# drprojects/superpoint_transformer

Measured on AMD Instinct MI355X. Metric: Mpoints/s SPT fwd+bwd on S3DIS-scale NAG, higher is better.
Workload: dtype f32 (the reference's shipped matmul class - configs/train.yaml:60-61 `float32_matmul_precision: high` = TF32 / bf16x3 next to `precision: 32` - as bf16x3: matrix products on the bf16 pipe with split operands, attention and the backward of the fused layers and of the attention blocks' Linears hi*hi +

## Files before the change

### superpoint_transformer_amd/csrc/fused_pool.hip

```cpp
#include <math.h>

#include <type_traits>

#include "common.hpp"

namespace spt {
namespace fpool {

typedef float f32x4 __attribute__((ext_vector_type(4)));
typedef __bf16 bf16x8 __attribute__((ext_vector_type(8)));
typedef __bf16 bf16x4 __attribute__((ext_vector_type(4)));
typedef short s16x4 __attribute__((ext_vector_type(4)));
#ifndef SPT_FPOOL_SKIP
#define SPT_FPOOL_SKIP 0
#endif
#ifndef SPT_FPOOL_WPAD
#define SPT_FPOOL_WPAD 16
#endif
constexpr int TR = 16;
constexpr int NWF = 8;
constexpr int ARG_NONE = 0x7fffffff;

__device__ __forceinline__ double xg_sum_d(double v) {
  v += __shfl_xor(v, 16, 64);
  v += __shfl_xor(v, 32, 64);
  return v;
}
__device__ __forceinline__ float xg_sum_f(float v) {
  v += __shfl_xor(v, 16, 64);
  v += __shfl_xor(v, 32, 64);
  return v;
}
__device__ __forceinline__ void wave_sync_lds() {
  __builtin_amdgcn_fence(__ATOMIC_RELEASE, "wavefront");
  __builtin_amdgcn_wave_barrier();
  __builtin_amdgcn_fence(__ATOMIC_ACQUIRE, "wavefront");
}
template <bool B16>
__device__ __forceinline__ float4 ld4(const float* __restrict__ base, int64_t elem) {
  if constexpr (B16) {
    const uint2 u = *reinterpret_cast<const uint2*>(reinterpret_cast<const uint16_t*>(base) + elem);
    return make_float4(__uint_as_float(u.x << 16), __uint_as_float(u.x & 0xffff0000u),
                       __uint_as_float(u.y << 16), __uint_as_float(u.y & 0xffff0000u));
  } else {
    return *reinterpret_cast<const float4*>(base + elem);
  }
}
template <int NV, typename V>
__device__ __forceinline__ void split2(const float (&x)[NV], V& hi, V& lo) {
#pragma unroll
  for (int i = 0; i < NV; ++i) {
    const __bf16 h = (__bf16)x[i];
    hi[i] = h;
    lo[i] = (__bf16)(x[i] - (float)h);
  }
}
template <int NV, typename V>
__device__ __forceinline__ void split3(const float (&x)[NV], V& h, V& m, V& l) {
#pragma unroll
  for (int i = 0; i < NV; ++i) {
    const __bf16 a = (__bf16)x[i];
    const float r1 = x[i] - (float)a;
    const __bf16 b = (__bf16)r1;
    const float r2 = r1 - (float)b;
    h[i] = a;
    m[i] = b;
    l[i] = (__bf16)r2;
  }
}
__device__ __forceinline__ f32x4 mfma16(const bf16x4& a, const bf16x4& b, f32x4 c) {
  return __builtin_amdgcn_mfma_f32_16x16x16bf16_1k(__builtin_bit_cast(s16x4, a),
                                                   __builtin_bit_cast(s16x4, b), c, 0, 0, 0);
}

template <bool X16>
struct RowChunk { typedef float4 type; };
template <>
struct RowChunk<true> { typedef uint2 type; };
template <bool X16>
__device__ __forceinline__ float4 widen(const typename RowChunk<X16>::type& u) {
  if constexpr (X16) {
    return make_float4(__uint_as_float(u.x << 16), __uint_as_float(u.x & 0xffff0000u),
                       __uint_as_float(u.y << 16), __uint_as_float(u.y & 0xffff0000u));
  } else {
    return u;
  }
}
template <int K, bool X16>
__device__ __forceinline__ void load_rows(const float* __restrict__ x, int rid_l,
                                          typename RowChunk<X16>::type (&v)[TR * (K / 4) / 64], int lane) {
  constexpr int CH = K / 4, NIT = TR * CH / 64;
  static_assert(TR * CH % 64 == 0, "whole waves of chunks");
#pragma unroll
  for (int j = 0; j < NIT; ++j) {
    const int q = lane + 64 * j, rr = q / CH, k = (q - rr * CH) << 2;
// ... 132 lines not shown
  };

  const int64_t nw = (int64_t)gridDim.x * NWF, w = (int64_t)blockIdx.x * NWF + wid;
  const int64_t per = (((r1 - r0 + nw - 1) / nw) + TR - 1) / TR * TR;
  const int64_t pa0 = cut_at(r0 + w * per, r0, r1, pos_seg, rowptr);
  const int64_t pb0 = (w == nw - 1) ? r1 : cut_at(r0 + (w + 1) * per, r0, r1, pos_seg, rowptr);
  const bool has_rows = pa0 < pb0;
  const int64_t plast = pb0 - 1;
  auto ids_of = [&](int64_t p, int& rid, int& sg) {
    int64_t q = p + (lane & (TR - 1));
    q = q < plast ? q : plast;
    rid = perm ? perm[q] : (int)q;
    sg = pos_seg[q];
  };
  if (has_rows) {
  int seg_a, seg_b, rid_c, seg_c;
  typename RowChunk<IN16>::type xv[TR * (K / 4) / 64];
  {
    int rid0, rid1;
    ids_of(pa0, rid0, seg_a);
    load_rows<K, IN16>(x, rid0, xv, lane);
    ids_of(pa0 + TR, rid1, seg_b);
    ids_of(pa0 + 2 * TR, rid_c, seg_c);
    wave_sync_lds();
    store_rows<K, LDA, true, IN16>(xv, (int)((pb0 - pa0) < TR ? (pb0 - pa0) : TR), tab, pslope, al, lane);
    load_rows<K, IN16>(x, rid1, xv, lane);
  }
  for (int64_t p = pa0; p < pb0; p += TR) {
    const int cnt = (int)((pb0 - p) < TR ? (pb0 - p) : TR);
    wave_sync_lds();
    f32x4 C[NBK];
#pragma unroll
    for (int nb = 0; nb < NBK; ++nb) C[nb] = (f32x4){0.f, 0.f, 0.f, 0.f};
    if constexpr (!(SPT_FPOOL_SKIP & 4)) {
      constexpr int NSTEP = KS * NBK;
      constexpr int LA = NPL == 3 ? 2 : (NPL == 2 ? 3 : 6);
      bf16x8 wf[LA + 1][NPL];
      auto ldw = [&](int step, bf16x8 (&w)[NPL]) {
        const int ks = step / NBK, nb = step - ks * NBK;
        const int wo = (16 * nb + c) * LDW + 32 * ks + 8 * g;
#pragma unroll
        for (int pl = 0; pl < NPL; ++pl) w[pl] = *reinterpret_cast<const bf16x8*>(&wpl[pl][wo]);
      };
#pragma unroll
      for (int i = 0; i < LA; ++i) ldw(i, wf[i]);
      bf16x8 x1, x2, x3;
#pragma unroll
      for (int step = 0; step < NSTEP; ++step) {
        const int ks = step / NBK, nb = step - ks * NBK;
        if (nb == 0) {
          const float4 a0 = *reinterpret_cast<const float4*>(al + c * LDA + 32 * ks + 8 * g);
          const float4 a1 = *reinterpret_cast<const float4*>(al + c * LDA + 32 * ks + 8 * g + 4);
          const float av[8] = {a0.x, a0.y, a0.z, a0.w, a1.x, a1.y, a1.z, a1.w};
          if constexpr (PREC == 3) {
            split3<8>(av, x1, x2, x3);
          } else if constexpr (PREC == 2) {
            split2<8>(av, x1, x2);
          } else {
#pragma unroll
            for (int i = 0; i < 8; ++i) x1[i] = (__bf16)av[i];
          }
        }
        if (step + LA < NSTEP) ldw(step + LA, wf[(step + LA) % (LA + 1)]);
        __builtin_amdgcn_sched_barrier(0);
        const bf16x8 (&w)[NPL] = wf[step % (LA + 1)];
        f32x4 acc = C[nb];
        if constexpr (PREC == 3) {
          acc = __builtin_amdgcn_mfma_f32_16x16x32_bf16(x3, w[0], acc, 0, 0, 0);
          acc = __builtin_amdgcn_mfma_f32_16x16x32_bf16(x1, w[NPL - 1], acc, 0, 0, 0);
          acc = __builtin_amdgcn_mfma_f32_16x16x32_bf16(x2, w[NPL > 1 ? 1 : 0], acc, 0, 0, 0);
          acc = __builtin_amdgcn_mfma_f32_16x16x32_bf16(x2, w[0], acc, 0, 0, 0);
          acc = __builtin_amdgcn_mfma_f32_16x16x32_bf16(x1, w[NPL > 1 ? 1 : 0], acc, 0, 0, 0);
        } else if constexpr (PREC == 2) {
          acc = __builtin_amdgcn_mfma_f32_16x16x32_bf16(x2, w[0], acc, 0, 0, 0);
          acc = __builtin_amdgcn_mfma_f32_16x16x32_bf16(x1, w[NPL - 1], acc, 0, 0, 0);
        }
        acc = __builtin_amdgcn_mfma_f32_16x16x32_bf16(x1, w[0], acc, 0, 0, 0);
        C[nb] = acc;
        __builtin_amdgcn_sched_barrier(0);
      }
    }
    if constexpr (!(SPT_FPOOL_SKIP & 1)) {
      bf16x4 Yh[KB], Yl[KB];
#pragma unroll
      for (int kb = 0; kb < KB; ++kb) {
        float yv[4];
#pragma unroll
        for (int r = 0; r < 4; ++r) yv[r] = al[(4 * g + r) * LDA + 16 * kb + c];
        if constexpr (PREC != 1) {
          const float sh = tab[3 * K + 16 * kb + c];
#pragma unroll
          for (int r = 0; r < 4; ++r) yv[r] = (4 * g + r < cnt) ? yv[r] - sh : 0.f;
        }
        if constexpr (PREC == 1) {
#pragma unroll
          for (int r = 0; r < 4; ++r) {
            Yh[kb][r] = (__bf16)yv[r];
            yv[r] = (float)Yh[kb][r];
          }
        } else {
          split2<4>(yv, Yh[kb], Yl[kb]);
        }
        sy[kb] += (yv[0] + yv[1]) + (yv[2] + yv[3]);
      }
      int gi = 0;
#pragma unroll
      for (int mi = 0; mi < KB; ++mi)
#pragma unroll
        for (int ni = mi; ni < KB; ++ni) {
          f32x4 acc = GA[gi];
          if constexpr (PREC != 1) {
            acc = mfma16(Yl[mi], Yl[ni], acc);
            acc = mfma16(Yl[mi], Yh[ni], acc);
            acc = mfma16(Yh[mi], Yl[ni], acc);
          }
          GA[gi] = mfma16(Yh[mi], Yh[ni], acc);
          ++gi;
        }
    }
    wave_sync_lds();
    {
      const int64_t left = pb0 - (p + TR);
      store_rows<K, LDA, true, IN16>(xv, (int)(left < 0 ? 0 : (left < TR ? left : TR)), tab, pslope, al, lane);
      asm volatile("" : "+v"(rid_c), "+v"(seg_c));
    }
    const int seg_cur = seg_a;
    if constexpr (!(SPT_FPOOL_SKIP & 2)) {
      const int pos0 = (int)p + 4 * g;
      int row = 0;
      while (row < cnt) {
        const int s = __builtin_amdgcn_readlane(seg_cur, row);
        const uint64_t diff = __ballot(lane < cnt && lane > row && seg_cur != s);
        const int e = diff ? (int)__builtin_ctzll(diff) : cnt;
        if (s != cur_seg) {
          if (cur_seg >= 0) flush(cur_seg);
          cur_seg = s;
        }
        if (row == 0 && e == TR) {
#pragma unroll
          for (int r = 0; r < 4; ++r)
#pragma unroll
            for (int nb = 0; nb < NBK; ++nb) {
              const float v = C[nb][r];
              const bool win = v > pm[nb];
              pm[nb] = win ? v : pm[nb];
              pp[nb] = win ? pos0 + r : pp[nb];
            }
        } else {
#pragma unroll
          for (int r = 0; r < 4; ++r) {
            const int rr = 4 * g + r;
            const bool in = rr >= row && rr < e;
#pragma unroll
            for (int nb = 0; nb < NBK; ++nb) {
              const float v = in ? C[nb][r] : -INFINITY;
              const bool win = v > pm[nb];
              pm[nb] = win ? v : pm[nb];
              pp[nb] = win ? pos0 + r : pp[nb];
            }
          }
        }
        row = e;
      }
    }
    load_rows<K, IN16>(x, rid_c, xv, lane);
    seg_a = seg_b;
    seg_b = seg_c;
    ids_of(p + 3 * TR, rid_c, seg_c);
  }
  }
  if (cur_seg >= 0) flush(cur_seg);

  for (int i = threadIdx.x; i < K * K + K; i += NWF * 64) gred[i] = 0.0;
  __syncthreads();
  for (int ww = 0; ww < NWF; ++ww) {
// ... 164 lines not shown
    const float* __restrict__ sc, const float* __restrict__ bs, float slope,
    const float* __restrict__ c1, float* __restrict__ gm) {
  const int64_t t4 = ((int64_t)blockIdx.x * blockDim.x + threadIdx.x) * 4;
  if (t4 >= num_seg * N) return;
  const int64_t s = t4 / N;
  const int c = (int)(t4 - s * N);
  const int64_t gph = seg_graph ? seg_graph[s] : 0;
  const float4 go = *reinterpret_cast<const float4*>(gout + t4);
  const float4 hv = *reinterpret_cast<const float4*>(raw + t4);
  const float4 a = *reinterpret_cast<const float4*>(am + gph * N + c);
  const float4 sv = *reinterpret_cast<const float4*>(sc + gph * N + c);
  const float4 b = *reinterpret_cast<const float4*>(bs + c);
  const float4 k1 = *reinterpret_cast<const float4*>(c1 + gph * N + c);
  const float gg[4] = {go.x, go.y, go.z, go.w}, hh[4] = {hv.x, hv.y, hv.z, hv.w};
  const float aa[4] = {a.x, a.y, a.z, a.w}, ss[4] = {sv.x, sv.y, sv.z, sv.w};
  const float bb[4] = {b.x, b.y, b.z, b.w}, q1[4] = {k1.x, k1.y, k1.z, k1.w};
  float o[4];
#pragma unroll
  for (int e = 0; e < 4; ++e) {
    float g_ = gg[e];
    if (slope != 1.f) {
      const float y = fmaf(hh[e] - aa[e], ss[e], bb[e]);
      g_ = (y > 0.f) ? g_ : g_ * slope;
    }
    o[e] = q1[e] * g_;
  }
  *reinterpret_cast<float4*>(gm + t4) = make_float4(o[0], o[1], o[2], o[3]);
}

template <int K>
__global__ __launch_bounds__(256) void pool_bwd_coef_kernel(
    const float* __restrict__ W, int N, const float* __restrict__ am, const float* __restrict__ c2,
    const float* __restrict__ c3, float* __restrict__ M, float* __restrict__ c0) {
  const int b = blockIdx.x;
  extern __shared__ float sm[];
  float* Bc = sm;
  float* Ac = sm + N;
  for (int i = threadIdx.x; i < N; i += blockDim.x) {
    const float k2 = c2[b * N + i];
    Bc[i] = -k2;
    Ac[i] = fmaf(k2, am[b * N + i], -c3[b * N + i]);
  }
  __syncthreads();
  for (int i = blockIdx.y * blockDim.x + threadIdx.x; i < K * K + K; i += gridDim.y * blockDim.x) {
    double acc = 0.0;
    if (i < K * K) {
      const int j = i / K, k = i - j * K;
      for (int c = 0; c < N; ++c)
        acc += (double)W[(size_t)c * K + j] * (double)Bc[c] * (double)W[(size_t)c * K + k];
      M[(size_t)b * K * K + i] = (float)acc;
    } else {
      const int k = i - K * K;
      for (int c = 0; c < N; ++c) acc += (double)Ac[c] * (double)W[(size_t)c * K + k];
      c0[(size_t)b * K + k] = (float)acc;
    }
  }
}

template <int K>
__global__ __launch_bounds__(256) void pool_bwd_gw_dense_kernel(
    const double* __restrict__ gram, int B, const float* __restrict__ W, int N, int bfw,
    const float* __restrict__ am, const float* __restrict__ c2, const float* __restrict__ c3,
    float* __restrict__ gW) {
  constexpr int GLEN = K * K + K + 1;
  const int t = blockIdx.x * blockDim.x + threadIdx.x;
  if (t >= N * K) return;
  const int c = t / K, k = t - c * K;
  double acc = 0.0;
  for (int b = 0; b < B; ++b) {
    const double* gr = gram + (size_t)b * GLEN;
    const double k2 = (double)c2[b * N + c];
    const double Ac = (double)fmaf(c2[b * N + c], am[b * N + c], -c3[b * N + c]);
    double t1 = 0.0;
    for (int j = 0; j < K; ++j) {
      float w = W[(size_t)c * K + j];
      if (bfw) w = (float)(__bf16)w;
      t1 += (double)w * gr[j * K + k];
    }
    acc += -k2 * t1 + Ac * gr[K * K + k];
  }
  gW[t] = (float)((double)gW[t] + acc);
}

template <int K, int N, bool LO, bool X16, int NW>
__global__ __launch_bounds__(NW * 64, NW / 4) void bwd_pool_kernel(
    const float* __restrict__ gm, const int32_t* __restrict__ argpos,
    const int32_t* __restrict__ perm, const int32_t* __restrict__ pos_seg,
    const float* __restrict__ xprev, const float* __restrict__ pam,
    const float* __restrict__ psc, const float* __restrict__ pbs, float pslope,
    const float* __restrict__ W, const float* __restrict__ Mg, const float* __restrict__ c0g,
    float* __restrict__ gx, float* __restrict__ gw_partial, double* __restrict__ pstat_partial,
    FmlpRuns rt) {
  constexpr int KB = K / 16, NBK = N / 16, NS = N / 32, KS = K / 32;
  constexpr int NBH = NBK / 2, KBH = KB / 2;
  constexpr int LDG = N + 4, LDX = K + 4;
  constexpr int LDT = N + SPT_FPOOL_WPAD, LDM = K + SPT_FPOOL_WPAD;
  static_assert((LDT % 32 == 16 && LDM % 32 == 16) || SPT_FPOOL_WPAD != 16, "conflict-free B fragments");
  constexpr int CPL = N / 64;
  static_assert(K % 32 == 0 && N % 64 == 0 && NW % 2 == 0, "shape");
  __shared__ __attribute__((aligned(16))) float g_lds[NW][TR * LDG];
  __shared__ __attribute__((aligned(16))) float x_lds[NW][TR * LDX];
  __shared__ __attribute__((aligned(16))) __bf16 wt_hi[K * LDT];
  __shared__ __attribute__((aligned(16))) __bf16 wt_lo[LO ? K * LDT : 8];
  __shared__ __attribute__((aligned(16))) __bf16 mt_hi[K * LDM];
  __shared__ __attribute__((aligned(16))) __bf16 mt_lo[LO ? K * LDM : 8];
  __shared__ __attribute__((aligned(16))) float pt[3 * K];
  __shared__ __attribute__((aligned(16))) float c0l[K];
  const int lane = threadIdx.x & 63;
  const int wid = __builtin_amdgcn_readfirstlane(threadIdx.x >> 6);
  const int hf = wid & 1;
  const int nb0 = hf * NBH, kb0 = hf * KBH;
  const int g = lane >> 4, c = lane & 15;
  const int run = blockIdx.y, gph = rt.g[run];
  const int64_t r0 = rt.r0[run], r1 = rt.r1[run];
  pam += (size_t)gph * K;
  psc += (size_t)gph * K;
  Mg += (size_t)gph * K * K;
  c0g += (size_t)gph * K;
  constexpr int SCR = 4 * (K / 32) * 64;
  float* gw_scratch = gw_partial + (size_t)gridDim.y * gridDim.x * N * K +
                      (size_t)run * gridDim.x * (NW / 2) * 2 * SCR;
  gw_partial += (size_t)run * gridDim.x * N * K;
  pstat_partial += (size_t)run * gridDim.x * (NW / 2) * (2 * K + 1);
  float* gl = g_lds[wid];
  float* xl = x_lds[wid];
  for (int i = threadIdx.x; i < K * N; i += NW * 64) {
    const int k = i / N, n = i - k * N;
    const float w = W[(size_t)n * K + k];
    const __bf16 hh = (__bf16)w;
    wt_hi[k * LDT + n] = hh;
    if constexpr (LO) wt_lo[k * LDT + n] = (__bf16)(w - (float)hh);
  }
  for (int i = threadIdx.x; i < K * K; i += NW * 64) {
    const int k = i / K, j = i - k * K;
    const float m = Mg[(size_t)j * K + k];
    const __bf16 hh = (__bf16)m;
    mt_hi[k * LDM + j] = hh;
    if constexpr (LO) mt_lo[k * LDM + j] = (__bf16)(m - (float)hh);
  }
  for (int i = threadIdx.x; i < K; i += NW * 64) {
    pt[i] = pam[i];
    pt[K + i] = psc[i];
    pt[2 * K + i] = pbs[i];
    c0l[i] = c0g[i];
  }
  __syncthreads();

  f32x4 C3[NBH][KB];
#pragma unroll
  for (int nb = 0; nb < NBH; ++nb)
#pragma unroll
    for (int kb = 0; kb < KB; ++kb) C3[nb][kb] = (f32x4){0.f, 0.f, 0.f, 0.f};
  double p1[KBH], p2[KBH];
#pragma unroll
  for (int kb = 0; kb < KBH; ++kb) p1[kb] = p2[kb] = 0.0;

  const int64_t ntiles = (r1 - r0 + TR - 1) / TR;
  const int64_t pair = (int64_t)blockIdx.x * (NW / 2) + (wid >> 1);
  const int64_t npairs = (int64_t)gridDim.x * (NW / 2);
  auto cnt_of = [&](int64_t t) {
    const int64_t row0 = r0 + t * TR;
    return (t < ntiles) ? (int)((r1 - row0) < TR ? (r1 - row0) : TR) : 0;
  };
  auto load_ids = [&](int64_t t, int& rid, int& sg) {
    const int64_t tt = t < ntiles ? t : ntiles - 1;
    int64_t q = r0 + tt * TR + (lane & (TR - 1));
    q = q < r1 - 1 ? q : r1 - 1;
    rid = perm ? perm[q] : (int)q;
    sg = pos_seg[q];
  };
  auto load_seg = [&](int sgm, int (&ap)[CPL], float (&gv)[CPL]) {
    const size_t o = (size_t)sgm * N + CPL * lane;
    if constexpr (CPL == 2) {
      const int2 a2 = *reinterpret_cast<const int2*>(argpos + o);
      const float2 g2 = *reinterpret_cast<const float2*>(gm + o);
      ap[0] = a2.x; ap[1] = a2.y;
      gv[0] = g2.x; gv[1] = g2.y;
    } else {
      ap[0] = argpos[o];
      gv[0] = gm[o];
    }
  };
  auto scatter = [&](const int (&ap)[CPL], const float (&gv)[CPL], int row0i, int lo, int hi) {
#pragma unroll
    for (int q = 0; q < CPL; ++q) {
      const int rr = ap[q] - row0i;
      const bool ok = rr >= lo && rr < hi;
      gl[ok ? rr * LDG + CPL * lane + q : N + q] = gv[q];
    }
  };
  if (ntiles > 0) {
  int rid_l, seg_l, rid_n, seg_n;
  load_ids(pair, rid_l, seg_l);
  typename RowChunk<X16>::type xv[TR * (K / 4) / 64];
  load_rows<K, X16>(xprev, rid_l, xv, lane);
  int apA[CPL], apB[CPL];
  float gvA[CPL], gvB[CPL];
  {
    const int c0 = cnt_of(pair < ntiles ? pair : ntiles - 1);
    load_seg(__builtin_amdgcn_readlane(seg_l, 0), apA, gvA);
    load_seg(__builtin_amdgcn_readlane(seg_l, c0 - 1), apB, gvB);
  }
  load_ids(pair + npairs, rid_n, seg_n);
  {
    float* scratch = gw_scratch + ((size_t)pair * 2 + hf) * SCR;
#pragma unroll
    for (int i = 0; i < 4 * KBH; ++i) scratch[lane + 64 * i] = 0.f;
  }
  auto tile = [&](auto full_c, int64_t t) {
    constexpr bool FULL = decltype(full_c)::value;
    const int64_t row0 = r0 + t * TR;
    const int cnt = FULL ? TR : cnt_of(t);
    wave_sync_lds();
    store_rows<K, LDX, false, X16>(xv, cnt, nullptr, 1.f, xl, lane);
    {
      constexpr int NZ = TR * (N / 4) / 64;
#pragma unroll
      for (int j = 0; j < NZ; ++j) {
        const int q = lane + 64 * j, rr = q / (N / 4), n = (q - rr * (N / 4)) << 2;
        *reinterpret_cast<float4*>(gl + rr * LDG + n) = make_float4(0.f, 0.f, 0.f, 0.f);
      }
      const int sA = __builtin_amdgcn_readlane(seg_l, 0);
      const int sB = __builtin_amdgcn_readlane(seg_l, cnt - 1);
      const uint64_t notA = __ballot(lane < cnt && seg_l != sA);
      const int eA = notA ? (int)__builtin_ctzll(notA) : cnt;
      const uint64_t isB = __ballot(lane < cnt && seg_l == sB);
      const int bB = (int)__builtin_ctzll(isB);
      scatter(apA, gvA, (int)row0, 0, eA);
      if (sB != sA) scatter(apB, gvB, (int)row0, bB, cnt);
      int row = eA;
      while (row < bB) {
        const int sgm = __builtin_amdgcn_readlane(seg_l, row);
        const uint64_t diff = __ballot(lane < cnt && lane > row && seg_l != sgm);
        const int e = diff ? (int)__builtin_ctzll(diff) : cnt;
        int ap[CPL];
        float gv[CPL];
        load_seg(sgm, ap, gv);
        scatter(ap, gv, (int)row0, row, e);
        row = e;
      }
    }
    const int rid_cur = rid_l;
    load_rows<K, X16>(xprev, rid_n, xv, lane);
    {
      const int64_t tn = t + npairs < ntiles ? t + npairs : ntiles - 1;
      load_seg(__builtin_amdgcn_readlane(seg_n, 0), apA, gvA);
      load_seg(__builtin_amdgcn_readlane(seg_n, cnt_of(tn) - 1), apB, gvB);
    }
    rid_l = rid_n;
    seg_l = seg_n;
    load_ids(t + 2 * npairs, rid_n, seg_n);
    wave_sync_lds();
    auto ynorm = [&](float v, int k, bool ok) {
      v = fmaf(v - pt[k], pt[K + k], pt[2 * K + k]);
      v = (v > 0.f) ? v : v * pslope;
      return ok ? v : 0.f;
    };
    if constexpr (!(SPT_FPOOL_SKIP & 8)) {
      bf16x4 Xh[KB], Xl[KB];
#pragma unroll
      for (int kb = 0; kb < KB; ++kb) {
        const int k = 16 * kb + c;
        float xr4[4];
#pragma unroll
        for (int r = 0; r < 4; ++r) xr4[r] = ynorm(xl[(4 * g + r) * LDX + k], k, 4 * g + r < cnt);
        if constexpr (LO) {
          split2<4>(xr4, Xh[kb], Xl[kb]);
        } else {
#pragma unroll
          for (int r = 0; r < 4; ++r) Xh[kb][r] = (__bf16)xr4[r];
        }
      }
#pragma unroll
      for (int nb = 0; nb < NBH; ++nb) {
        float sv[4];
#pragma unroll
        for (int r = 0; r < 4; ++r) sv[r] = gl[(4 * g + r) * LDG + 16 * (nb0 + nb) + c];
        bf16x4 sh, sl;
        if constexpr (LO) {
          split2<4>(sv, sh, sl);
        } else {
#pragma unroll
          for (int r = 0; r < 4; ++r) sh[r] = (__bf16)sv[r];
        }
#pragma unroll
        for (int kb = 0; kb < KB; ++kb) {
          f32x4 acc = C3[nb][kb];
          if constexpr (LO) {
            acc = mfma16(sl, Xh[kb], acc);
            acc = mfma16(sh, Xl[kb], acc);
          }
          C3[nb][kb] = mfma16(sh, Xh[kb], acc);
        }
      }
    }
    {
      f32x4 CX[KBH];
#pragma unroll
      for (int kb = 0; kb < KBH; ++kb) {
        const float z = c0l[16 * (kb0 + kb) + c];
        CX[kb] = (f32x4){z, z, z, z};
      }
      constexpr int NPLB = LO ? 2 : 1, LAB = 2;
      constexpr int NST1 = NS * KBH, NST = NST1 + KS * KBH;
      bf16x8 bf[LAB + 1][NPLB];
      auto ldb = [&](int step, bf16x8 (&b)[NPLB]) {
        if (step < NST1) {
          const int sg = step / KBH, kb = step - sg * KBH;
          const int wo = (16 * (kb0 + kb) + c) * LDT + 32 * sg + 8 * g;
          b[0] = *reinterpret_cast<const bf16x8*>(wt_hi + wo);
          if constexpr (LO) b[NPLB - 1] = *reinterpret_cast<const bf16x8*>(wt_lo + wo);
        } else {
          const int st = step - NST1, ks = st / KBH, kb = st - ks * KBH;
          const int mo = (16 * (kb0 + kb) + c) * LDM + 32 * ks + 8 * g;
          b[0] = *reinterpret_cast<const bf16x8*>(mt_hi + mo);
          if constexpr (LO) b[NPLB - 1] = *reinterpret_cast<const bf16x8*>(mt_lo + mo);
        }
      };
#pragma unroll
      for (int i = 0; i < LAB; ++i) ldb(i, bf[i]);
      bf16x8 ah, alo;
#pragma unroll
      for (int step = 0; step < ((SPT_FPOOL_SKIP & 16) ? 0 : NST); ++step) {
        const bool first = step < NST1;
        const int sub = first ? step : step - NST1;
        const int blk = sub / KBH, kb = sub - blk * KBH;
        if (kb == 0) {
          float av[8];
          if (first) {
            const float4 a0 = *reinterpret_cast<const float4*>(gl + c * LDG + 32 * blk + 8 * g);
            const float4 a1 = *reinterpret_cast<const float4*>(gl + c * LDG + 32 * blk + 8 * g + 4);
            av[0] = a0.x; av[1] = a0.y; av[2] = a0.z; av[3] = a0.w;
            av[4] = a1.x; av[5] = a1.y; av[6] = a1.z; av[7] = a1.w;
          } else {
            const float4 a0 = *reinterpret_cast<const float4*>(xl + c * LDX + 32 * blk + 8 * g);
            const float4 a1 = *reinterpret_cast<const float4*>(xl + c * LDX + 32 * blk + 8 * g + 4);
            const float rv[8] = {a0.x, a0.y, a0.z, a0.w, a1.x, a1.y, a1.z, a1.w};
#pragma unroll
            for (int i = 0; i < 8; ++i) av[i] = ynorm(rv[i], 32 * blk + 8 * g + i, c < cnt);
          }
          if constexpr (LO) {
            split2<8>(av, ah, alo);
          } else {
#pragma unroll
            for (int i = 0; i < 8; ++i) ah[i] = (__bf16)av[i];
          }
        }
        if (step + LAB < NST) ldb(step + LAB, bf[(step + LAB) % (LAB + 1)]);
        __builtin_amdgcn_sched_barrier(0);
        const bf16x8 (&b)[NPLB] = bf[step % (LAB + 1)];
        f32x4 acc = CX[kb];
        if constexpr (LO) {
          acc = __builtin_amdgcn_mfma_f32_16x16x32_bf16(alo, b[0], acc, 0, 0, 0);
          acc = __builtin_amdgcn_mfma_f32_16x16x32_bf16(ah, b[NPLB - 1], acc, 0, 0, 0);
        }
        CX[kb] = __builtin_amdgcn_mfma_f32_16x16x32_bf16(ah, b[0], acc, 0, 0, 0);
        __builtin_amdgcn_sched_barrier(0);
      }
#pragma unroll
      for (int r = 0; r < 4; ++r) {
        const int rr = 4 * g + r;
        const int64_t orow = (int64_t)__shfl(rid_cur, rr, 64);
        if (FULL || rr < cnt) {
#pragma unroll
          for (int kb = 0; kb < KBH; ++kb) {
            const int k = 16 * (kb0 + kb) + c;
            const float v = CX[kb][r];
            gx[orow * K + k] = v;
            const float o = xl[rr * LDX + k] - pt[k];
            float gg = v;
            if (pslope != 1.f) {
              const float y = fmaf(o, pt[K + k], pt[2 * K + k]);
              gg = (y > 0.f) ? gg : gg * pslope;
            }
            if constexpr (!(SPT_FPOOL_SKIP & 32)) {
              p1[kb] += (double)gg;
              p2[kb] += (double)gg * (double)o;
            }
          }
        }
      }
    }
  };
  const int64_t nfull = (r1 - r0) / TR;
  int64_t t = pair;
  for (; t < nfull; t += npairs) tile(std::true_type{}, t);
  if (t < ntiles) tile(std::false_type{}, t);
  }
  double* pp = pstat_partial + (size_t)pair * (2 * K + 1);
#pragma unroll
  for (int kb = 0; kb < KBH; ++kb) {
    const double a = xg_sum_d(p1[kb]), b = xg_sum_d(p2[kb]);
    const int k = 16 * (kb0 + kb) + c;
    if (g == 0) {
      pp[k] = a;
      pp[K + k] = b;
    }
  }
  if (lane == 0 && hf == 0) pp[2 * K] = (pair == 0) ? (double)(r1 - r0) : 0.0;
  {
    constexpr int LDR = K + 4;
    static_assert(N * LDR <= NW * TR * LDG, "the table fits the S-tile buffers");
    const int pr = wid >> 1;
    __syncthreads();
    float* red = &g_lds[0][0];
#pragma unroll 1
    for (int p = 1; p < NW / 2; ++p) {
      if (pr == p) {
#pragma unroll
        for (int nb = 0; nb < NBH; ++nb)
#pragma unroll
          for (int kb = 0; kb < KB; ++kb)
#pragma unroll
            for (int r = 0; r < 4; ++r)
              red[(16 * (nb0 + nb) + 4 * g + r) * LDR + 16 * kb + c] = C3[nb][kb][r];
      }
      __syncthreads();
      if (pr == 0) {
#pragma unroll
        for (int nb = 0; nb < NBH; ++nb)
#pragma unroll
          for (int kb = 0; kb < KB; ++kb)
#pragma unroll
            for (int r = 0; r < 4; ++r)
              C3[nb][kb][r] += red[(16 * (nb0 + nb) + 4 * g + r) * LDR + 16 * kb + c];
      }
      __syncthreads();
    }
    if (pr == 0) {
      float* gwp = gw_partial + (size_t)blockIdx.x * N * K;
#pragma unroll
      for (int nb = 0; nb < NBH; ++nb)
#pragma unroll
        for (int kb = 0; kb < KB; ++kb)
#pragma unroll
          for (int r = 0; r < 4; ++r)
            gwp[(size_t)(16 * (nb0 + nb) + 4 * g + r) * K + 16 * kb + c] = C3[nb][kb][r];
    }
  }
}

}

#define SPT_FPOOL_SHAPES(X) X(64, 128) X(64, 64) X(32, 64)

bool fpool_supported(int K, int N) {
#define X(k, n) if (K == k && N == n) return true;
  SPT_FPOOL_SHAPES(X)
#undef X
  return false;
}
int fpool_gram_len(int K) { return K * K + K + 1; }

int fpool_fwd_blocks(int64_t max_rows, int nruns) {
  int64_t blocks = (max_rows + fpool::TR * fpool::NWF * 4 - 1) / (fpool::TR * fpool::NWF * 4);
  int64_t cap = 256 / nruns;
  if (cap < 1) cap = 1;
  if (blocks > cap) blocks = cap;
  return (int)(blocks < 1 ? 1 : blocks);
}

int fpool_fwd_launch(int prec, bool in16, const float* x, const int32_t* perm, const int32_t* pos_seg,
                     const int32_t* rowptr, const FmlpRuns& rt, int64_t max_rows, int K, int N,
                     const float* W, const float* gnw, const float* pam, const float* psc,
                     const float* pbs, float pslope, float* raw, int32_t* argpos, double* partial,
                     hipStream_t stream) {
  const int gx_ = fpool_fwd_blocks(max_rows, rt.n);
  const dim3 grid((unsigned)gx_, (unsigned)rt.n);
#define X(k, n)                                                                                   \
  if (K == k && N == n) {                                                                         \
    if (prec == 3 && !in16)                                                                       \
      fpool::fwd_pool_kernel<k, n, 3, false><<<grid, fpool::NWF * 64, 0, stream>>>(               \
          x, perm, pos_seg, rowptr, W, gnw, pam, psc, pbs, pslope, raw, argpos, partial, rt);        \
    else if (prec == 2 && !in16)                                                                  \
      fpool::fwd_pool_kernel<k, n, 2, false><<<grid, fpool::NWF * 64, 0, stream>>>(               \
          x, perm, pos_seg, rowptr, W, gnw, pam, psc, pbs, pslope, raw, argpos, partial, rt);        \
    else if (prec == 1 && !in16)                                                                  \
      fpool::fwd_pool_kernel<k, n, 1, false><<<grid, fpool::NWF * 64, 0, stream>>>(               \
          x, perm, pos_seg, rowptr, W, gnw, pam, psc, pbs, pslope, raw, argpos, partial, rt);        \
    else if (prec == 1 && in16)                                                                   \
      fpool::fwd_pool_kernel<k, n, 1, true><<<grid, fpool::NWF * 64, 0, stream>>>(                \
          x, perm, pos_seg, rowptr, W, gnw, pam, psc, pbs, pslope, raw, argpos, partial, rt);        \
    else                                                                                          \
      return -1;                                                                                  \
  }
  SPT_FPOOL_SHAPES(X)
#undef X
  return gx_;
// ... 91 lines not shown
```

Baseline: 349.6.

## Store scattered pool gradient tile as split bf16 in LDS and read with transpose loads

The backward pool kernel used to scatter gradients into an fp32 LDS tile and re-split them into bf16 hi/lo on every read. It now splits once at scatter time into adjacent hi/lo bf16 halves of each row and reads fragments with ds_read_tr16_b64 transpose loads. In the C3 accumulation, the two correction MFMAs become one K=32 MFMA over concatenated lo/hi operands. A small forward tweak also replaces a row-masking select with an FMA against a row-valid factor. These cut LDS bytes, conversion ALU work and MFMA count, at the cost of a new LDS layout and reliance on the transpose-load intrinsic.

```diff
diff --git a/superpoint_transformer_amd/csrc/fused_pool.hip b/superpoint_transformer_amd/csrc/fused_pool.hip
--- a/superpoint_transformer_amd/csrc/fused_pool.hip
+++ b/superpoint_transformer_amd/csrc/fused_pool.hip
@@ -11,6 +11,7 @@
 typedef __bf16 bf16x8 __attribute__((ext_vector_type(8)));
 typedef __bf16 bf16x4 __attribute__((ext_vector_type(4)));
 typedef short s16x4 __attribute__((ext_vector_type(4)));
+typedef __attribute__((address_space(3))) s16x4 lds_s16x4;
 #ifndef SPT_FPOOL_SKIP
 #define SPT_FPOOL_SKIP 0
 #endif
@@ -309,6 +310,9 @@
     }
     if constexpr (!(SPT_FPOOL_SKIP & 1)) {
       bf16x4 Yh[KB], Yl[KB];
+      float rowin[4];
+#pragma unroll
+      for (int r = 0; r < 4; ++r) rowin[r] = (4 * g + r < cnt) ? 1.f : 0.f;
 #pragma unroll
       for (int kb = 0; kb < KB; ++kb) {
         float yv[4];
@@ -317,7 +321,7 @@
         if constexpr (PREC != 1) {
           const float sh = tab[3 * K + 16 * kb + c];
 #pragma unroll
-          for (int r = 0; r < 4; ++r) yv[r] = (4 * g + r < cnt) ? yv[r] - sh : 0.f;
+          for (int r = 0; r < 4; ++r) yv[r] = fmaf(-sh, rowin[r], yv[r]);
         }
         if constexpr (PREC == 1) {
 #pragma unroll
@@ -659,12 +663,14 @@
     FmlpRuns rt) {
   constexpr int KB = K / 16, NBK = N / 16, NS = N / 32, KS = K / 32;
   constexpr int NBH = NBK / 2, KBH = KB / 2;
-  constexpr int LDG = N + 4, LDX = K + 4;
+  constexpr int LDX = K + 4;
   constexpr int LDT = N + SPT_FPOOL_WPAD, LDM = K + SPT_FPOOL_WPAD;
   static_assert((LDT % 32 == 16 && LDM % 32 == 16) || SPT_FPOOL_WPAD != 16, "conflict-free B fragments");
+  constexpr int NPS = LO ? 2 : 1, LDS_ = NPS * N + 16;
+  static_assert(LDS_ % 32 == 16, "conflict-free S reads");
   constexpr int CPL = N / 64;
   static_assert(K % 32 == 0 && N % 64 == 0 && NW % 2 == 0, "shape");
-  __shared__ __attribute__((aligned(16))) float g_lds[NW][TR * LDG];
+  __shared__ __attribute__((aligned(16))) __bf16 s_lds[NW][TR * LDS_];
   __shared__ __attribute__((aligned(16))) float x_lds[NW][TR * LDX];
   __shared__ __attribute__((aligned(16))) __bf16 wt_hi[K * LDT];
   __shared__ __attribute__((aligned(16))) __bf16 wt_lo[LO ? K * LDT : 8];
@@ -688,7 +694,7 @@
                       (size_t)run * gridDim.x * (NW / 2) * 2 * SCR;
   gw_partial += (size_t)run * gridDim.x * N * K;
   pstat_partial += (size_t)run * gridDim.x * (NW / 2) * (2 * K + 1);
-  float* gl = g_lds[wid];
+  __bf16* sl_ = s_lds[wid];
   float* xl = x_lds[wid];
   for (int i = threadIdx.x; i < K * N; i += NW * 64) {
     const int k = i / N, n = i - k * N;
@@ -752,7 +758,10 @@
     for (int q = 0; q < CPL; ++q) {
       const int rr = ap[q] - row0i;
       const bool ok = rr >= lo && rr < hi;
-      gl[ok ? rr * LDG + CPL * lane + q : N + q] = gv[q];
+      const int o = ok ? rr * LDS_ + CPL * lane + q : NPS * N + 2 * q;
+      const __bf16 h = (__bf16)gv[q];
+      sl_[o] = h;
+      if constexpr (LO) sl_[o + (ok ? N : 1)] = (__bf16)(gv[q] - (float)h);
     }
   };
   if (ntiles > 0) {
@@ -780,11 +789,11 @@
     wave_sync_lds();
     store_rows<K, LDX, false, X16>(xv, cnt, nullptr, 1.f, xl, lane);
     {
-      constexpr int NZ = TR * (N / 4) / 64;
+      constexpr int CHR = NPS * N / 8, NZ = TR * CHR / 64;
 #pragma unroll
       for (int j = 0; j < NZ; ++j) {
-        const int q = lane + 64 * j, rr = q / (N / 4), n = (q - rr * (N / 4)) << 2;
-        *reinterpret_cast<float4*>(gl + rr * LDG + n) = make_float4(0.f, 0.f, 0.f, 0.f);
+        const int q = lane + 64 * j, rr = q / CHR, n = (q - rr * CHR) << 3;
+        *reinterpret_cast<uint4*>(sl_ + rr * LDS_ + n) = make_uint4(0u, 0u, 0u, 0u);
       }
       const int sA = __builtin_amdgcn_readlane(seg_l, 0);
       const int sB = __builtin_amdgcn_readlane(seg_l, cnt - 1);
@@ -837,26 +846,31 @@
           for (int r = 0; r < 4; ++r) Xh[kb][r] = (__bf16)xr4[r];
         }
       }
+      bf16x8 XX[LO ? KB : 1];
+      if constexpr (LO) {
+#pragma unroll
+        for (int kb = 0; kb < KB; ++kb)
+          XX[kb] = __builtin_shufflevector(Xh[kb], Xl[kb], 0, 1, 2, 3, 4, 5, 6, 7);
+      }
+      const __bf16* str = sl_ + (4 * g + (c >> 2)) * LDS_ + 4 * (c & 3);
+      auto tr_read = [&](int off) {
+        return __builtin_bit_cast(bf16x4, __builtin_amdgcn_ds_read_tr16_b64_v4i16(
+            (lds_s16x4*)(__attribute__((address_space(3))) void*)(str + off)));
+      };
 #pragma unroll
       for (int nb = 0; nb < NBH; ++nb) {
-        float sv[4];
-#pragma unroll
-        for (int r = 0; r < 4; ++r) sv[r] = gl[(4 * g + r) * LDG + 16 * (nb0 + nb) + c];
-        bf16x4 sh, sl;
+        const bf16x4 sh = tr_read(16 * (nb0 + nb));
         if constexpr (LO) {
-          split2<4>(sv, sh, sl);
+          const bf16x4 slo = tr_read(N + 16 * (nb0 + nb));
+          const bf16x8 SS = __builtin_shufflevector(slo, sh, 0, 1, 2, 3, 4, 5, 6, 7);
+#pragma unroll
+          for (int kb = 0; kb < KB; ++kb) {
+            const f32x4 acc = __builtin_amdgcn_mfma_f32_16x16x32_bf16(SS, XX[kb], C3[nb][kb], 0, 0, 0);
+            C3[nb][kb] = mfma16(sh, Xh[kb], acc);
+          }
         } else {
 #pragma unroll
-          for (int r = 0; r < 4; ++r) sh[r] = (__bf16)sv[r];
-        }
-#pragma unroll
-        for (int kb = 0; kb < KB; ++kb) {
-          f32x4 acc = C3[nb][kb];
-          if constexpr (LO) {
-            acc = mfma16(sl, Xh[kb], acc);
-            acc = mfma16(sh, Xl[kb], acc);
-          }
-          C3[nb][kb] = mfma16(sh, Xh[kb], acc);
+          for (int kb = 0; kb < KB; ++kb) C3[nb][kb] = mfma16(sh, Xh[kb], C3[nb][kb]);
         }
       }
     }
@@ -892,24 +906,23 @@
         const int sub = first ? step : step - NST1;
         const int blk = sub / KBH, kb = sub - blk * KBH;
         if (kb == 0) {
-          float av[8];
           if (first) {
-            const float4 a0 = *reinterpret_cast<const float4*>(gl + c * LDG + 32 * blk + 8 * g);
-            const float4 a1 = *reinterpret_cast<const float4*>(gl + c * LDG + 32 * blk + 8 * g + 4);
-            av[0] = a0.x; av[1] = a0.y; av[2] = a0.z; av[3] = a0.w;
-            av[4] = a1.x; av[5] = a1.y; av[6] = a1.z; av[7] = a1.w;
+            const __bf16* sr = sl_ + c * LDS_ + 32 * blk + 8 * g;
+            ah = *reinterpret_cast<const bf16x8*>(sr);
+            if constexpr (LO) alo = *reinterpret_cast<const bf16x8*>(sr + N);
           } else {
             const float4 a0 = *reinterpret_cast<const float4*>(xl + c * LDX + 32 * blk + 8 * g);
             const float4 a1 = *reinterpret_cast<const float4*>(xl + c * LDX + 32 * blk + 8 * g + 4);
             const float rv[8] = {a0.x, a0.y, a0.z, a0.w, a1.x, a1.y, a1.z, a1.w};
+            float av[8];
 #pragma unroll
             for (int i = 0; i < 8; ++i) av[i] = ynorm(rv[i], 32 * blk + 8 * g + i, c < cnt);
-          }
-          if constexpr (LO) {
-            split2<8>(av, ah, alo);
-          } else {
-#pragma unroll
-            for (int i = 0; i < 8; ++i) ah[i] = (__bf16)av[i];
+            if constexpr (LO) {
+              split2<8>(av, ah, alo);
+            } else {
+#pragma unroll
+              for (int i = 0; i < 8; ++i) ah[i] = (__bf16)av[i];
+            }
           }
         }
         if (step + LAB < NST) ldb(step + LAB, bf[(step + LAB) % (LAB + 1)]);
@@ -966,10 +979,10 @@
   if (lane == 0 && hf == 0) pp[2 * K] = (pair == 0) ? (double)(r1 - r0) : 0.0;
   {
     constexpr int LDR = K + 4;
-    static_assert(N * LDR <= NW * TR * LDG, "the table fits the S-tile buffers");
+    static_assert(2 * N * LDR <= NW * TR * LDS_, "the table fits the S-tile buffers");
     const int pr = wid >> 1;
     __syncthreads();
-    float* red = &g_lds[0][0];
+    float* red = reinterpret_cast<float*>(&s_lds[0][0]);
 #pragma unroll 1
     for (int p = 1; p < NW / 2; ++p) {
       if (pr == p) {
```

Measured after the change: 353.6, median of 6. 1.2% higher.

## Share pre-split bf16 tile planes between wave pairs via LDS flags in pool backward

Applied to the files above, without the earlier changes.

The backward pool kernel now has the two waves of a pair split the staging of each tile: each wave loads half the rows and half the channels, normalizes and splits them into swizzled bf16 hi/lo planes in a shared per-pair LDS record, and the pair synchronizes through LDS flag spin-waits. The MFMA operands are then read with ds_read_tr16 transpose loads, and hi/lo pairs are packed into a single 16x16x32 MFMA plus a 16x16x16 one, replacing three separate 16x16x16 MFMAs. The aim is to cut the redundant per-wave fp32 staging, the repeated ynorm and split work, and the LDS footprint. In exchange it adds inter-wave spin synchronization, with a trap if a wait times out, and it rounds S to bf16 before the MFMAs.

```diff
diff --git a/superpoint_transformer_amd/csrc/fused_pool.hip b/superpoint_transformer_amd/csrc/fused_pool.hip
--- a/superpoint_transformer_amd/csrc/fused_pool.hip
+++ b/superpoint_transformer_amd/csrc/fused_pool.hip
@@ -648,6 +648,36 @@
   gW[t] = (float)((double)gW[t] + acc);
 }
 
+typedef __attribute__((address_space(3))) s16x4 lds_s16x4;
+typedef __attribute__((address_space(3))) volatile int lds_flag_t;
+__device__ __forceinline__ void flag_set(lds_flag_t* f, int v) {
+  asm volatile("s_waitcnt lgkmcnt(0)" ::: "memory");
+  *f = v;
+}
+__device__ __forceinline__ bool flag_wait(lds_flag_t* f, int v) {
+  int spins = 0;
+  bool ok = true;
+#pragma clang loop unroll(disable)
+  while (__builtin_amdgcn_readfirstlane(*f) < v) {
+    __builtin_amdgcn_s_sleep(1);
+    if (++spins > (1 << 22)) {
+      ok = false;
+      break;
+    }
+  }
+  asm volatile("" ::: "memory");
+  return ok;
+}
+template <int C>
+__device__ __forceinline__ int pl_off(int row, int col) {
+  constexpr int RPL = 128 / C;
+  static_assert(C == 32 || C == 64 || C == 128, "plane row of 64, 128 or 256 bytes");
+  const int swz = ((row / RPL) & (8 / RPL - 1)) << 1;
+  return row * C + ((((col >> 3) ^ swz) << 3) | (col & 7));
+}
+__device__ __forceinline__ s16x4 tr_read(const __bf16* p) {
+  return __builtin_amdgcn_ds_read_tr16_b64_v4i16((lds_s16x4*)(__attribute__((address_space(3))) void*)p);
+}
 template <int K, int N, bool LO, bool X16, int NW>
 __global__ __launch_bounds__(NW * 64, NW / 4) void bwd_pool_kernel(
     const float* __restrict__ gm, const int32_t* __restrict__ argpos,
@@ -659,13 +689,27 @@
     FmlpRuns rt) {
   constexpr int KB = K / 16, NBK = N / 16, NS = N / 32, KS = K / 32;
   constexpr int NBH = NBK / 2, KBH = KB / 2;
-  constexpr int LDG = N + 4, LDX = K + 4;
+  constexpr int LDX = K + 4;
   constexpr int LDT = N + SPT_FPOOL_WPAD, LDM = K + SPT_FPOOL_WPAD;
   static_assert((LDT % 32 == 16 && LDM % 32 == 16) || SPT_FPOOL_WPAD != 16, "conflict-free B fragments");
-  constexpr int CPL = N / 64;
   static_assert(K % 32 == 0 && N % 64 == 0 && NW % 2 == 0, "shape");
-  __shared__ __attribute__((aligned(16))) float g_lds[NW][TR * LDG];
-  __shared__ __attribute__((aligned(16))) float x_lds[NW][TR * LDX];
+  constexpr int NP = NW / 2, NPL = LO ? 2 : 1;
+  constexpr int HR = TR / 2;
+  constexpr int CH = K / 4, NIT = HR * CH / 64;
+  static_assert(HR * CH % 64 == 0, "whole waves of chunks");
+  constexpr int NH = N / 2;
+  static_assert(NH <= 64 && (NH & (NH - 1)) == 0, "one channel per lane");
+  constexpr int NZ = TR * (NH / 8) / 64;
+  static_assert(TR * (NH / 8) % 64 == 0, "whole waves of chunks");
+  constexpr int T_X = 0;
+  constexpr int T_Y = T_X + TR * LDX * 4;
+  constexpr int T_S = T_Y + NPL * TR * K * 2;
+  constexpr int T_PAD = T_S + NPL * TR * N * 2;
+  constexpr int T_FLAG = T_PAD + 16;
+  constexpr int T_END = T_FLAG + 16;
+  static_assert(T_Y % 16 == 0 && T_END % 16 == 0, "16-byte chunks");
+  constexpr int F_STAGED = 0, F_DONE = 2;
+  __shared__ __attribute__((aligned(16))) unsigned char tile_lds[NP * T_END];
   __shared__ __attribute__((aligned(16))) __bf16 wt_hi[K * LDT];
   __shared__ __attribute__((aligned(16))) __bf16 wt_lo[LO ? K * LDT : 8];
   __shared__ __attribute__((aligned(16))) __bf16 mt_hi[K * LDM];
@@ -688,8 +732,12 @@
                       (size_t)run * gridDim.x * (NW / 2) * 2 * SCR;
   gw_partial += (size_t)run * gridDim.x * N * K;
   pstat_partial += (size_t)run * gridDim.x * (NW / 2) * (2 * K + 1);
-  float* gl = g_lds[wid];
-  float* xl = x_lds[wid];
+  unsigned char* tl = tile_lds + (wid >> 1) * T_END;
+  float* xr = reinterpret_cast<float*>(tl + T_X);
+  __bf16* yp = reinterpret_cast<__bf16*>(tl + T_Y);
+  __bf16* sp = reinterpret_cast<__bf16*>(tl + T_S);
+  __bf16* pad = reinterpret_cast<__bf16*>(tl + T_PAD);
+  lds_flag_t* flg = (lds_flag_t*)(__attribute__((address_space(3))) void*)(tl + T_FLAG);
   for (int i = threadIdx.x; i < K * N; i += NW * 64) {
     const int k = i / N, n = i - k * N;
     const float w = W[(size_t)n * K + k];
@@ -710,6 +758,7 @@
     pt[2 * K + i] = pbs[i];
     c0l[i] = c0g[i];
   }
+  if (lane < 4) flg[lane] = 0;
   __syncthreads();
 
   f32x4 C3[NBH][KB];
@@ -735,33 +784,39 @@
     rid = perm ? perm[q] : (int)q;
     sg = pos_seg[q];
   };
-  auto load_seg = [&](int sgm, int (&ap)[CPL], float (&gv)[CPL]) {
-    const size_t o = (size_t)sgm * N + CPL * lane;
-    if constexpr (CPL == 2) {
-      const int2 a2 = *reinterpret_cast<const int2*>(argpos + o);
-      const float2 g2 = *reinterpret_cast<const float2*>(gm + o);
-      ap[0] = a2.x; ap[1] = a2.y;
-      gv[0] = g2.x; gv[1] = g2.y;
-    } else {
-      ap[0] = argpos[o];
-      gv[0] = gm[o];
+  auto load_half = [&](int rid, typename RowChunk<X16>::type (&v)[NIT]) {
+#pragma unroll
+    for (int j = 0; j < NIT; ++j) {
+      const int q = lane + 64 * j, rl = q / CH, k = (q - rl * CH) << 2;
+      const int64_t xrow = (int64_t)__shfl(rid, HR * hf + rl, 64);
+      if constexpr (X16)
+        v[j] = *reinterpret_cast<const uint2*>(reinterpret_cast<const uint16_t*>(xprev) + xrow * K + k);
+      else
+        v[j] = *reinterpret_cast<const float4*>(xprev + xrow * K + k);
     }
   };
-  auto scatter = [&](const int (&ap)[CPL], const float (&gv)[CPL], int row0i, int lo, int hi) {
-#pragma unroll
-    for (int q = 0; q < CPL; ++q) {
-      const int rr = ap[q] - row0i;
-      const bool ok = rr >= lo && rr < hi;
-      gl[ok ? rr * LDG + CPL * lane + q : N + q] = gv[q];
-    }
+  const int chn = hf * NH + (lane & (NH - 1));
+  const bool sc_on = lane < NH;
+  auto load_seg = [&](int sgm, int& ap, float& gv) {
+    const size_t o = (size_t)sgm * N + chn;
+    ap = argpos[o];
+    gv = gm[o];
+  };
+  auto scatter = [&](int ap, float gv, int row0i, int lo, int hi) {
+    const int rr = ap - row0i;
+    const bool ok = sc_on && rr >= lo && rr < hi;
+    const int o = pl_off<N>(rr & (TR - 1), chn);
+    const __bf16 h = (__bf16)gv;
+    *(ok ? sp + o : pad) = h;
+    if constexpr (LO) *(ok ? sp + TR * N + o : pad + 1) = (__bf16)(gv - (float)h);
   };
   if (ntiles > 0) {
   int rid_l, seg_l, rid_n, seg_n;
   load_ids(pair, rid_l, seg_l);
-  typename RowChunk<X16>::type xv[TR * (K / 4) / 64];
-  load_rows<K, X16>(xprev, rid_l, xv, lane);
-  int apA[CPL], apB[CPL];
-  float gvA[CPL], gvB[CPL];
+  typename RowChunk<X16>::type xv[NIT];
+  load_half(rid_l, xv);
+  int apA, apB;
+  float gvA, gvB;
   {
     const int c0 = cnt_of(pair < ntiles ? pair : ntiles - 1);
     load_seg(__builtin_amdgcn_readlane(seg_l, 0), apA, gvA);
@@ -773,18 +828,46 @@
 #pragma unroll
     for (int i = 0; i < 4 * KBH; ++i) scratch[lane + 64 * i] = 0.f;
   }
+  int kseq = 0;
+  bool lost = false;
   auto tile = [&](auto full_c, int64_t t) {
     constexpr bool FULL = decltype(full_c)::value;
     const int64_t row0 = r0 + t * TR;
     const int cnt = FULL ? TR : cnt_of(t);
-    wave_sync_lds();
-    store_rows<K, LDX, false, X16>(xv, cnt, nullptr, 1.f, xl, lane);
+    auto ynorm = [&](float v, int k, bool ok) {
+      v = fmaf(v - pt[k], pt[K + k], pt[2 * K + k]);
+      v = (v > 0.f) ? v : v * pslope;
+      return ok ? v : 0.f;
+    };
+    if (!lost) lost = !flag_wait(flg + F_DONE + (hf ^ 1), kseq);
+#pragma unroll
+    for (int j = 0; j < NIT; ++j) {
+      const int q = lane + 64 * j, rl = q / CH, k = (q - rl * CH) << 2, rr = HR * hf + rl;
+      const bool ok = rr < cnt;
+      float4 w = widen<X16>(xv[j]);
+      if (!ok) w = make_float4(0.f, 0.f, 0.f, 0.f);
+      *reinterpret_cast<float4*>(xr + rr * LDX + k) = w;
+      const float yv[4] = {ynorm(w.x, k, ok), ynorm(w.y, k + 1, ok), ynorm(w.z, k + 2, ok),
+                           ynorm(w.w, k + 3, ok)};
+      bf16x4 yh, yl;
+      const int o = pl_off<K>(rr, k);
+      if constexpr (LO) {
+        split2<4>(yv, yh, yl);
+        *reinterpret_cast<bf16x4*>(yp + TR * K + o) = yl;
+      } else {
+#pragma unroll
+        for (int i = 0; i < 4; ++i) yh[i] = (__bf16)yv[i];
+      }
+      *reinterpret_cast<bf16x4*>(yp + o) = yh;
+    }
     {
-      constexpr int NZ = TR * (N / 4) / 64;
 #pragma unroll
       for (int j = 0; j < NZ; ++j) {
-        const int q = lane + 64 * j, rr = q / (N / 4), n = (q - rr * (N / 4)) << 2;
-        *reinterpret_cast<float4*>(gl + rr * LDG + n) = make_float4(0.f, 0.f, 0.f, 0.f);
+        const int q = lane + 64 * j, rr = q / (NH / 8), ch = hf * (NH / 8) + (q - rr * (NH / 8));
+        const int o = pl_off<N>(rr, 8 * ch);
+        const bf16x8 z = __builtin_bit_cast(bf16x8, make_uint4(0u, 0u, 0u, 0u));
+        *reinterpret_cast<bf16x8*>(sp + o) = z;
+        if constexpr (LO) *reinterpret_cast<bf16x8*>(sp + TR * N + o) = z;
       }
       const int sA = __builtin_amdgcn_readlane(seg_l, 0);
       const int sB = __builtin_amdgcn_readlane(seg_l, cnt - 1);
@@ -799,15 +882,15 @@
         const int sgm = __builtin_amdgcn_readlane(seg_l, row);
         const uint64_t diff = __ballot(lane < cnt && lane > row && seg_l != sgm);
         const int e = diff ? (int)__builtin_ctzll(diff) : cnt;
-        int ap[CPL];
-        float gv[CPL];
+        int ap;
+        float gv;
         load_seg(sgm, ap, gv);
         scatter(ap, gv, (int)row0, row, e);
         row = e;
       }
     }
     const int rid_cur = rid_l;
-    load_rows<K, X16>(xprev, rid_n, xv, lane);
+    load_half(rid_n, xv);
     {
       const int64_t tn = t + npairs < ntiles ? t + npairs : ntiles - 1;
       load_seg(__builtin_amdgcn_readlane(seg_n, 0), apA, gvA);
@@ -816,56 +899,48 @@
     rid_l = rid_n;
     seg_l = seg_n;
     load_ids(t + 2 * npairs, rid_n, seg_n);
-    wave_sync_lds();
-    auto ynorm = [&](float v, int k, bool ok) {
-      v = fmaf(v - pt[k], pt[K + k], pt[2 * K + k]);
-      v = (v > 0.f) ? v : v * pslope;
-      return ok ? v : 0.f;
-    };
+    flag_set(flg + F_STAGED + hf, kseq + 1);
+    if (!lost) lost = !flag_wait(flg + F_STAGED + (hf ^ 1), kseq + 1);
     if constexpr (!(SPT_FPOOL_SKIP & 8)) {
-      bf16x4 Xh[KB], Xl[KB];
+      const int trow = 4 * g + (c >> 2), tcol = 4 * (c & 3);
+      s16x4 Xh[KB];
+      bf16x8 Xc[LO ? KB : 1];
 #pragma unroll
       for (int kb = 0; kb < KB; ++kb) {
-        const int k = 16 * kb + c;
-        float xr4[4];
-#pragma unroll
-        for (int r = 0; r < 4; ++r) xr4[r] = ynorm(xl[(4 * g + r) * LDX + k], k, 4 * g + r < cnt);
+        const __bf16* p = yp + pl_off<K>(trow, 16 * kb + tcol);
+        Xh[kb] = tr_read(p);
+        if constexpr (LO)
+          Xc[kb] = __builtin_bit_cast(bf16x8, __builtin_shufflevector(Xh[kb], tr_read(p + TR * K),
+                                                                      0, 1, 2, 3, 4, 5, 6, 7));
+      }
+#pragma unroll
+      for (int nb = 0; nb < NBH; ++nb) {
+        const __bf16* p = sp + pl_off<N>(trow, 16 * (nb0 + nb) + tcol);
+        const s16x4 sh = tr_read(p);
         if constexpr (LO) {
-          split2<4>(xr4, Xh[kb], Xl[kb]);
+          const s16x4 sl = tr_read(p + TR * N);
+          const bf16x8 Sc = __builtin_bit_cast(bf16x8, __builtin_shufflevector(sl, sh, 0, 1, 2, 3, 4, 5, 6, 7));
+#pragma unroll
+          for (int kb = 0; kb < KB; ++kb) {
+            const f32x4 acc = __builtin_amdgcn_mfma_f32_16x16x32_bf16(Sc, Xc[kb], C3[nb][kb], 0, 0, 0);
+            C3[nb][kb] = __builtin_amdgcn_mfma_f32_16x16x16bf16_1k(sh, Xh[kb], acc, 0, 0, 0);
+          }
         } else {
 #pragma unroll
-          for (int r = 0; r < 4; ++r) Xh[kb][r] = (__bf16)xr4[r];
-        }
-      }
-#pragma unroll
-      for (int nb = 0; nb < NBH; ++nb) {
-        float sv[4];
-#pragma unroll
-        for (int r = 0; r < 4; ++r) sv[r] = gl[(4 * g + r) * LDG + 16 * (nb0 + nb) + c];
-        bf16x4 sh, sl;
-        if constexpr (LO) {
-          split2<4>(sv, sh, sl);
-        } else {
-#pragma unroll
-          for (int r = 0; r < 4; ++r) sh[r] = (__bf16)sv[r];
-        }
-#pragma unroll
-        for (int kb = 0; kb < KB; ++kb) {
-          f32x4 acc = C3[nb][kb];
-          if constexpr (LO) {
-            acc = mfma16(sl, Xh[kb], acc);
-            acc = mfma16(sh, Xl[kb], acc);
-          }
-          C3[nb][kb] = mfma16(sh, Xh[kb], acc);
+          for (int kb = 0; kb < KB; ++kb)
+            C3[nb][kb] = __builtin_amdgcn_mfma_f32_16x16x16bf16_1k(sh, Xh[kb], C3[nb][kb], 0, 0, 0);
         }
       }
     }
     {
       f32x4 CX[KBH];
+      float xo[4][KBH];
 #pragma unroll
       for (int kb = 0; kb < KBH; ++kb) {
         const float z = c0l[16 * (kb0 + kb) + c];
         CX[kb] = (f32x4){z, z, z, z};
+#pragma unroll
+        for (int r = 0; r < 4; ++r) xo[r][kb] = xr[(4 * g + r) * LDX + 16 * (kb0 + kb) + c];
       }
       constexpr int NPLB = LO ? 2 : 1, LAB = 2;
       constexpr int NST1 = NS * KBH, NST = NST1 + KS * KBH;
@@ -892,25 +967,9 @@
         const int sub = first ? step : step - NST1;
         const int blk = sub / KBH, kb = sub - blk * KBH;
         if (kb == 0) {
-          float av[8];
-          if (first) {
-            const float4 a0 = *reinterpret_cast<const float4*>(gl + c * LDG + 32 * blk + 8 * g);
-            const float4 a1 = *reinterpret_cast<const float4*>(gl + c * LDG + 32 * blk + 8 * g + 4);
-            av[0] = a0.x; av[1] = a0.y; av[2] = a0.z; av[3] = a0.w;
-            av[4] = a1.x; av[5] = a1.y; av[6] = a1.z; av[7] = a1.w;
-          } else {
-            const float4 a0 = *reinterpret_cast<const float4*>(xl + c * LDX + 32 * blk + 8 * g);
-            const float4 a1 = *reinterpret_cast<const float4*>(xl + c * LDX + 32 * blk + 8 * g + 4);
-            const float rv[8] = {a0.x, a0.y, a0.z, a0.w, a1.x, a1.y, a1.z, a1.w};
-#pragma unroll
-            for (int i = 0; i < 8; ++i) av[i] = ynorm(rv[i], 32 * blk + 8 * g + i, c < cnt);
-          }
-          if constexpr (LO) {
-            split2<8>(av, ah, alo);
-          } else {
-#pragma unroll
-            for (int i = 0; i < 8; ++i) ah[i] = (__bf16)av[i];
-          }
+          const __bf16* p = first ? sp + pl_off<N>(c, 32 * blk + 8 * g) : yp + pl_off<K>(c, 32 * blk + 8 * g);
+          ah = *reinterpret_cast<const bf16x8*>(p);
+          if constexpr (LO) alo = *reinterpret_cast<const bf16x8*>(p + (first ? TR * N : TR * K));
         }
         if (step + LAB < NST) ldb(step + LAB, bf[(step + LAB) % (LAB + 1)]);
         __builtin_amdgcn_sched_barrier(0);
@@ -923,6 +982,7 @@
         CX[kb] = __builtin_amdgcn_mfma_f32_16x16x32_bf16(ah, b[0], acc, 0, 0, 0);
         __builtin_amdgcn_sched_barrier(0);
       }
+      flag_set(flg + F_DONE + hf, kseq + 1);
 #pragma unroll
       for (int r = 0; r < 4; ++r) {
         const int rr = 4 * g + r;
@@ -933,7 +993,7 @@
             const int k = 16 * (kb0 + kb) + c;
             const float v = CX[kb][r];
             gx[orow * K + k] = v;
-            const float o = xl[rr * LDX + k] - pt[k];
+            const float o = xo[r][kb] - pt[k];
             float gg = v;
             if (pslope != 1.f) {
               const float y = fmaf(o, pt[K + k], pt[2 * K + k]);
@@ -947,11 +1007,13 @@
         }
       }
     }
+    ++kseq;
   };
   const int64_t nfull = (r1 - r0) / TR;
   int64_t t = pair;
   for (; t < nfull; t += npairs) tile(std::true_type{}, t);
   if (t < ntiles) tile(std::false_type{}, t);
+  if (lost) __builtin_trap();
   }
   double* pp = pstat_partial + (size_t)pair * (2 * K + 1);
 #pragma unroll
@@ -966,10 +1028,10 @@
   if (lane == 0 && hf == 0) pp[2 * K] = (pair == 0) ? (double)(r1 - r0) : 0.0;
   {
     constexpr int LDR = K + 4;
-    static_assert(N * LDR <= NW * TR * LDG, "the table fits the S-tile buffers");
+    static_assert(N * LDR * 4 <= NP * T_END, "the table fits the tile records");
     const int pr = wid >> 1;
     __syncthreads();
-    float* red = &g_lds[0][0];
+    float* red = reinterpret_cast<float*>(tile_lds);
 #pragma unroll 1
     for (int p = 1; p < NW / 2; ++p) {
       if (pr == p) {
```

Result: faster. 344.5 before, 354.9 after (median of 6 runs) (+3.0%).
